# CloudEngineHub/PARC

Hardware: AMD Instinct MI355X
Metric: env-steps/s (higher is better)
Workload: dtype f32; 1 GPU; full step (dynamics + obs/reward/done), 65536 envs total = 65536 per GPU, 5 bundled clips on a square blocky grid, reset of finished envs included; envs_per_gpu=65536, total_envs=65536, dynamics=True, parallelism=env-shard x1, launch=stream launches, library_abi=6

## Files before the change

parc_amd/csrc/parc_env.hip:

```cpp
#include <hip/hip_runtime.h>

#include <cmath>
#include <cstddef>
#include <cstdio>
#include <cstring>
#include <new>
#include <string>
#include <vector>

#include "../../include/parc_env.h"
#include "parc_math.hpp"
#include "parc_dynamics.hpp"
#include "parc_dynamics_coop.hpp"
#include "parc_dynamics_wave.hpp"

using namespace parc;

#define REC_F4 32
#define REC_Q_POS 15
#define REC_Q_CONTACT 16
#define REC_Q_VEL 20

struct HierTables {
    float lt[16][3];
    float lr[16][4];
    int fk_paths[PARC_MAX_FK_PATHS][PARC_MAX_FK_DEPTH];
    int key_ids[8];
    int key_slot[16];
    int parent[16];
    int jtype[16];
    int dof_idx[16];
    float axis[16][4];
};
#define HIER_STAGED_WORDS ((int)(offsetof(HierTables, parent) / 4))

#define TILE_MAX_CELLS 320

struct DevTables {
    HierTables h;
    float tstep[8];
    float joint_err_w[16];
    float dof_err_w[PARC_MAX_DOFS];
    float contact_w[16];
    float pose_term_dist[16];
};

struct MotionMeta {
    int start, nframes;
    float length;
    int loop;
    float dx, dy, dz;
    float fps;
};

struct StepParams {
    int N, B, J, D, K, S, R, M, T;
    int lds_wave_floats;
    int global_obs, off_char;
    int lr_identity;
    int obs_tar, obs_contact;
    int obs_dim, off_dofvel, off_key, off_tar, tar_w, off_tarc, off_cc, off_hf;
    float dt_f, episode_length, min_obs_h, max_obs_h;
    float pose_w, vel_w, root_pos_w, root_vel_w, key_pos_w;
    float root_pos_term_sq, root_rot_term;
    int early_term, pose_term, track_root, track_root_h, tracking, body_pos_from_fk, never_done;
    unsigned fall_mask;
    float term_h;
    const float *hf; int X, Y; float min_x, min_y, dx, dy; int tile_r;
    float rdx, rdy;
    unsigned tile_mul;
    float tstep[8];
    const float4 *records; const MotionMeta *meta; const float *motion_offsets; const float *env_offsets;
    const float *ray_points; const DevTables *tables;
    unsigned char *ema_code;
    unsigned *stamp_out;
    float4 *prep;
    ParcEnvBuffers buf;
};

struct Blend { int i0, i1; float b; };

__device__ __forceinline__ Blend frame_blend(const MotionMeta &m, float t) {
    float phase = t / m.length;
    if (m.loop == PARC_LOOP_WRAP) phase = phase - floorf(phase);
    phase = fminf(fmaxf(phase, 0.f), 1.f);
    float pf = phase * (float)(m.nframes - 1);
    int f0 = (int)pf;
    f0 = max(0, min(f0, m.nframes - 1));
    int f1 = min(f0 + 1, m.nframes - 1);
    Blend r;
    r.b = pf - (float)f0;
    r.i0 = f0 + m.start;
    r.i1 = f1 + m.start;
    return r;
}

__device__ __forceinline__ Q4 joint_dof_to_rot(int type, const float *axis4, const float *dof) {
    if (type == PARC_JOINT_HINGE) return axis_angle_to_quat(mk3(axis4[0], axis4[1], axis4[2]), dof[0]);
    if (type == PARC_JOINT_SPHERICAL) return exp_map_to_quat(mk3(dof[0], dof[1], dof[2]));
    return mk4(0.f, 0.f, 0.f, 1.f);
}

__device__ __forceinline__ void joint_rot_to_dof(int type, const float *axis4, Q4 q, float *out) {
// ... 41 lines not shown

__global__ __launch_bounds__(64) void k_env_prep(const StepParams P, const int64_t *__restrict__ env_ids,
                                                 const int *__restrict__ env_ids32, const int *__restrict__ count_dev, int count) {
    if (count_dev) count = *count_dev;
    const int it = blockIdx.x * 4 + (threadIdx.x >> 4), j = threadIdx.x & 15;
    if (it >= count || j >= P.B) return;
    const int e = env_ids ? (int)env_ids[it] : (env_ids32 ? env_ids32[it] : it);
    const DevTables *__restrict__ T = P.tables;
    float4 *out = P.prep + (size_t)e * 16;
    if (j == 0) {
        const float4 rr = *(const float4 *)(P.buf.char_root_rot + 4 * (size_t)e);
        const float heading = calc_heading(rr);
        const Q4 hinv = heading_quat_inv(heading);
        out[0] = make_float4(cosf(heading), sinf(heading), hinv.z, hinv.w);
    } else {
        const float *dof = P.buf.char_dof_pos + (size_t)e * P.D;
        const int ty = T->h.jtype[j], di = T->h.dof_idx[j];
        Q4 q = mk4(0.f, 0.f, 0.f, 1.f);
        if (ty == PARC_JOINT_HINGE) q = axis_angle_to_quat(mk3(T->h.axis[j][0], T->h.axis[j][1], T->h.axis[j][2]), dof[di]);
        else if (ty == PARC_JOINT_SPHERICAL) q = exp_map_to_quat(mk3(dof[di], dof[di + 1], dof[di + 2]));
        out[j] = q;
    }
}

#ifdef PARC_STAMPS
#define STAMP(i) do { if (lane == 0) s_stamp[i] = __builtin_readcyclecounter(); } while (0)
#else
#define STAMP(i) do { } while (0)
#endif
#define MODE_STEP 0
#define MODE_OBS 1
#define ENVS_PER_BLOCK 4
#define WAVE_SYNC() asm volatile("" ::: "memory")
#define RAY_UNROLL 8

__device__ __forceinline__ float wave_sum(float v) {
#pragma unroll
    for (int off = 32; off >= 1; off >>= 1) v = v + __shfl_xor(v, off, 64);
    return v;
}

template <int CTRL>
__device__ __forceinline__ float dpp_f32(float v) {
    return __int_as_float(__builtin_amdgcn_update_dpp(0, __float_as_int(v), CTRL, 0xf, 0xf, false));
}
__device__ __forceinline__ float row_sum16(float v) {
    v = v + dpp_f32<0x128>(v);
    v = v + dpp_f32<0x124>(v);
    v = v + dpp_f32<0x122>(v);
    v = v + dpp_f32<0x121>(v);
    return v;
}
__device__ __forceinline__ float lane_value(float v, int l) { return __int_as_float(__builtin_amdgcn_readlane(__float_as_int(v), l)); }

template <int MODE, bool MIRROR, bool LOCALROOT = false, bool OBSVAR = false>
__global__ __launch_bounds__(256, 5) void k_env_post(const StepParams P, const int64_t *__restrict__ env_ids,
                                                 const int *__restrict__ env_ids32, const int *__restrict__ count_dev, int count,
                                                 unsigned long long *bump_calls) {
    extern __shared__ __align__(16) float s_obs_all[];
    __shared__ int s_tab_raw[HIER_STAGED_WORDS];
    const HierTables &s_tab = *reinterpret_cast<const HierTables *>(s_tab_raw);
    __shared__ float4 s_q_all[ENVS_PER_BLOCK][8][16];
    __shared__ float4 s_lq_all[ENVS_PER_BLOCK][2][16];
    __shared__ float4 s_fk_all[ENVS_PER_BLOCK][80];
    __shared__ float s_cdofv_all[ENVS_PER_BLOCK][PARC_MAX_DOFS];
    __shared__ float4 s_refvel_all[ENVS_PER_BLOCK][12];
    __shared__ float s_refct_all[ENVS_PER_BLOCK][16];
    __shared__ float s_cfn_all[ENVS_PER_BLOCK][16];
    __shared__ float s_sc_all[ENVS_PER_BLOCK][16];
#ifdef PARC_STAMPS
    __shared__ unsigned long long s_stamp_all[ENVS_PER_BLOCK][16];
#endif
    const int wv = __builtin_amdgcn_readfirstlane((int)(threadIdx.x >> 6));
    const int lane = threadIdx.x & 63;
    const bool GLOBALOBS = OBSVAR && P.global_obs != 0;
    const int oc = OBSVAR ? P.off_char : 0;
    const bool TAROBS = !OBSVAR || P.obs_tar != 0;
    const bool CONTACTOBS = !OBSVAR || P.obs_contact != 0;
    float *s_obs = s_obs_all + (size_t)wv * P.lds_wave_floats;
    float4 (*s_q)[16] = s_q_all[wv];
    float4 (*s_lq)[16] = s_lq_all[wv];
    float4 *s_fk = s_fk_all[wv];
    float4 *s_cbp = s_lq[0];
    float *s_cdofv = s_cdofv_all[wv];
    float4 *s_refvel = s_refvel_all[wv];
    float *s_refct = s_refct_all[wv], *s_cfn = s_cfn_all[wv];
#ifdef PARC_STAMPS
    unsigned long long *s_stamp = s_stamp_all[wv];
#endif
    float *s_tile = (float *)s_fk;
    float4 (*s_br)[16] = reinterpret_cast<float4 (*)[16]>(s_obs + ((P.off_tarc + 3) & ~3));

    if (MODE == MODE_OBS && bump_calls && blockIdx.x == 0 && threadIdx.x == 0) *bump_calls += 1ull;
    if (count_dev) count = *count_dev;
    const int it = blockIdx.x * ENVS_PER_BLOCK + wv;
    if (it >= count) return;
    int e = env_ids ? (int)env_ids[it] : (env_ids32 ? env_ids32[it] : it);
    e = __builtin_amdgcn_readfirstlane(e);
    STAMP(0);

    const int B = P.B, D = P.D, S = P.S, K = P.K, J = P.J;
    const DevTables *__restrict__ T = P.tables;

    float *orow = P.buf.obs + (size_t)e * P.obs_dim;

    constexpr int HW = HIER_STAGED_WORDS;
    constexpr int HN = (HW + 63) / 64;
    int tabreg[HN];
#pragma unroll
    for (int i = 0; i < HN; ++i) { const int w = lane + 64 * i; tabreg[i] = w < HW ? ((const int *)&T->h)[w] : 0; }
    float dofv = 0.f;
    if (lane < D) dofv = P.buf.char_dof_vel[(size_t)e * D + lane];
    float aux0 = 0.f, aux1 = 0.f, aux2 = 0.f;
    {
        const float *src = nullptr;
        if (lane >= 32 && lane < 32 + B) src = P.buf.contact_forces + 3 * ((size_t)e * B + (lane - 32));
        else if (lane == 30) src = P.buf.char_root_vel + 3 * (size_t)e;
        else if (lane == 31) src = P.buf.char_root_ang_vel + 3 * (size_t)e;
        if (src) { aux0 = src[0]; aux1 = src[1]; aux2 = src[2]; }
    }
    const int qi = lane & 15;
    float4 prepq = make_float4(0.f, 0.f, 0.f, 1.f);
    if (lane < 16) prepq = P.prep[(size_t)e * 16 + lane];
    float2 rayp[RAY_UNROLL];
#pragma unroll
    for (int i = 0; i < RAY_UNROLL; ++i) {
        const int r = lane + 64 * i;
        rayp[i] = r < P.R ? ((const float2 *)P.ray_points)[r] : make_float2(0.f, 0.f);
    }

    const int mid = P.buf.motion_ids[e];
    const int tid = P.buf.terrain_ids[e];
    const float toff = P.buf.time_offsets[e];
    int ts = P.buf.timestep[e];
    if (MODE == MODE_STEP) ts += 1;
    const float time = P.dt_f * (float)ts;
    const float mt = time + toff;
    const MotionMeta meta = P.meta[mid];
    const float eox = P.env_offsets[3 * e + 0], eoy = P.env_offsets[3 * e + 1], eoz = P.env_offsets[3 * e + 2];
    const float *mo = P.motion_offsets + 2 * ((size_t)mid * P.T + tid);
    const float offx = mo[0] - eox, offy = mo[1] - eoy;
    const float *crp = P.buf.char_root_pos + 3 * (size_t)e;
    const float *crr = P.buf.char_root_rot + 4 * (size_t)e;
    const V3 root_pos = mk3(crp[0], crp[1], crp[2]);
    const Q4 root_rot = mk4(crr[0], crr[1], crr[2], crr[3]);
    const float gx = root_pos.x + eox, gy = root_pos.y + eoy, gz = root_pos.z + eoz;

    Blend myb;
    {
        const int sid = lane & 7;
        float t = mt;
#pragma unroll
        for (int q = 0; q < PARC_MAX_TAR_STEPS; ++q) t = (sid - 1 == q) ? mt + P.tstep[q] : t;
        myb = frame_blend(meta, t);
    }
    const int last_frame = meta.start + meta.nframes - 1;
    float4 fA[2], fB[2];
    Blend bl[2];
#pragma unroll
    for (int p = 0; p < 2; ++p) {
        const int r = p * 4 + (lane >> 4);
        const int src = max(r - 1, 0);
        bl[p].b = __shfl(myb.b, src, 64);
        bl[p].i0 = __shfl(myb.i0, src, 64);
        bl[p].i1 = min(bl[p].i0 + 1, last_frame);
        fA[p] = make_float4(0.f, 0.f, 0.f, 1.f); fB[p] = fA[p];
        if (r >= 1 && r < 2 + S) {
            fA[p] = P.records[(size_t)bl[p].i0 * REC_F4 + qi];
            fB[p] = P.records[(size_t)bl[p].i1 * REC_F4 + qi];
        }
    }
    float4 cA = make_float4(0.f, 0.f, 0.f, 0.f), cB = cA;
    float cblend = 0.f;
    const int nvel = 2 + (D + 3) / 4;
    {
        const int src = lane < 4 * (1 + S) ? lane >> 2 : 0;
        const float b2b = __shfl(myb.b, src, 64);
        const int b2i0 = __shfl(myb.i0, src, 64), b2i1 = min(b2i0 + 1, last_frame);
        if (lane < 4 * (1 + S)) {
            const int c = lane & 3;
            cblend = b2b;
            cA = P.records[(size_t)b2i0 * REC_F4 + REC_Q_CONTACT + c];
            cB = P.records[(size_t)b2i1 * REC_F4 + REC_Q_CONTACT + c];
        } else if (lane >= 32 && lane < 32 + nvel) {
            cA = P.records[(size_t)b2i0 * REC_F4 + REC_Q_VEL + (lane - 32)];
        }
    }
    const int tr = P.tile_r, TW = 2 * tr + 1, ncell = tr >= 0 ? TW * TW : 0;
    const int ox = min(max(cell_index(gx, P.min_x, P.dx) - tr, -(1 << 22)), 1 << 22), oy = min(max(cell_index(gy, P.min_y, P.dy) - tr, -(1 << 22)), 1 << 22);
    float tilev[5];
#pragma unroll
    for (int i = 0; i < 5; ++i) {
        const int idx = lane + 64 * i;
        tilev[i] = 0.f;
        if (idx < ncell) {
            const int a = (int)(((unsigned)idx * P.tile_mul) >> 16), bq = idx - a * TW;
            const int cx = min(max(ox + a, 0), P.X - 1), cy = min(max(oy + bq, 0), P.Y - 1);
            tilev[i] = P.hf[(size_t)cx * P.Y + cy];
        }
    }

    const float ch = __shfl(prepq.x, 0, 64), sh = __shfl(prepq.y, 0, 64);
    const Q4 hinv = mk4(0.f, 0.f, __shfl(prepq.z, 0, 64), __shfl(prepq.w, 0, 64));
#pragma unroll
    for (int i = 0; i < HN; ++i) { const int w = lane + 64 * i; if (w < HW) s_tab_raw[w] = tabreg[i]; }
    if (lane < D) {
        s_cdofv[lane] = dofv;
        s_obs[P.off_dofvel + lane] = dofv;
    }
    if (OBSVAR && oc && lane == 29) s_obs[0] = root_pos.z;
    if (lane == 30 || lane == 31) {
        const V3 r = GLOBALOBS ? mk3(aux0, aux1, aux2) : quat_rotate(hinv, mk3(aux0, aux1, aux2));
        const int o = oc + (lane == 30 ? 6 : 9);
        s_obs[o + 0] = r.x; s_obs[o + 1] = r.y; s_obs[o + 2] = r.z;
    }
    if (lane >= 32 && lane < 32 + B) {
        const float n = norm3(mk3(aux0, aux1, aux2));
        if (CONTACTOBS) orow[P.off_cc + (lane - 32)] = n > 1e-5f ? 1.f : 0.f;
        s_cfn[lane - 32] = fminf(n, 1.0f);
    }
#pragma unroll
    for (int i = 0; i < 5; ++i) { const int idx = lane + 64 * i; if (idx < ncell) s_tile[idx] = tilev[i]; }
    WAVE_SYNC();
    STAMP(1);

    {
        float *hrow = orow + P.off_hf;
        float *hmirror = MIRROR && P.buf.ray_hfs ? P.buf.ray_hfs + (size_t)e * P.R : nullptr;
        for (int base = 0; base < P.R; base += 64 * RAY_UNROLL) {
            if (base > 0) {
#pragma unroll
                for (int i = 0; i < RAY_UNROLL; ++i) { const int r = base + lane + 64 * i; rayp[i] = r < P.R ? ((const float2 *)P.ray_points)[r] : make_float2(0.f, 0.f); }
            }
            const float tlox = (float)ox, thix = (float)(ox + TW - 1), tloy = (float)oy, thiy = (float)(oy + TW - 1);
            if (tr >= 0) {
                int tix[RAY_UNROLL];
#pragma unroll
                for (int i = 0; i < RAY_UNROLL; ++i) {
                    tix[i] = 0;
                    if (base + 64 * i < P.R) {
                        const float px = (rayp[i].x * ch - rayp[i].y * sh) + gx;
                        const float py = (rayp[i].x * sh + rayp[i].y * ch) + gy;
                        const int a = (int)fminf(fmaxf(cell_float_rcp(px, P.min_x, P.dx, P.rdx), tlox), thix) - ox;
                        const int bq = (int)fminf(fmaxf(cell_float_rcp(py, P.min_y, P.dy, P.rdy), tloy), thiy) - oy;
                        tix[i] = a * TW + bq;
                    }
                    asm volatile("" : "+v"(tix[i]));
                }
                float hv[RAY_UNROLL];
#pragma unroll
                for (int i = 0; i < RAY_UNROLL; ++i) hv[i] = s_tile[tix[i]];
#pragma unroll
                for (int i = 0; i < RAY_UNROLL; ++i) {
                    const int r = base + lane + 64 * i;
                    if (r < P.R) {
                        float h = hv[i] - gz;
                        h = fminf(fmaxf(h, P.min_obs_h), P.max_obs_h);
                        hrow[r] = h;
                        if (hmirror) hmirror[r] = h;
                    }
                }
            } else {
#pragma unroll
                for (int i = 0; i < RAY_UNROLL; ++i) {
                    const int r = base + lane + 64 * i;
                    if (r < P.R) {
                        const float px = (rayp[i].x * ch - rayp[i].y * sh) + gx;
                        const float py = (rayp[i].x * sh + rayp[i].y * ch) + gy;
                        const int ix = cell_index_rcp(px, P.min_x, P.dx, P.rdx), iy = cell_index_rcp(py, P.min_y, P.dy, P.rdy);
                        const int cx = min(max(ix, 0), P.X - 1), cy = min(max(iy, 0), P.Y - 1);
                        float h = P.hf[(size_t)cx * P.Y + cy] - gz;
                        h = fminf(fmaxf(h, P.min_obs_h), P.max_obs_h);
                        hrow[r] = h;
                        if (hmirror) hmirror[r] = h;
                    }
                }
            }
        }
    }
    STAMP(2);

#pragma unroll
    for (int p = 0; p < 2; ++p) {
        const int r = p * 4 + (lane >> 4);
        const int i = qi;
        if (r < 2 + S) {
            float4 res = make_float4(0.f, 0.f, 0.f, 1.f);
            if (r == 0) {
                if (i == 0) res = root_rot;
                else if (i == 15) res = make_float4(root_pos.x, root_pos.y, root_pos.z, 0.f);
                else if (i < B) res = prepq;
            } else {
                const float4 A = fA[p], Bv = fB[p];
                const float bb = bl[p].b;
                if (i == 15) {
                    const float a = 1.0f - bb;
                    res.x = a * A.x + bb * Bv.x;
                    res.y = a * A.y + bb * Bv.y;
                    res.z = a * A.z + bb * Bv.z;
                    res.w = 0.f;
                    if (meta.loop == PARC_LOOP_WRAP) {
                        float t = mt;
#pragma unroll
                        for (int q = 0; q < PARC_MAX_TAR_STEPS; ++q) t = (r - 2 == q) ? mt + P.tstep[q] : t;
                        const float ph = floorf(t / meta.length);
                        res.x = res.x + ph * meta.dx; res.y = res.y + ph * meta.dy; res.z = res.z + ph * meta.dz;
                    }
                    res.x = res.x + offx;
                    res.y = res.y + offy;
                } else if (i < B) {
                    res = slerp_rr(A, Bv, bb);
                }
// ... 327 lines not shown
                te[3] = pe / (float)B;
                te[4] = dve / (float)D;
                te[5] = (fabsf(tv.x - rvx) + fabsf(tv.y - rvy) + fabsf(tv.z - rvz)) / 3.f;
                te[6] = (fabsf(tav.x - rax) + fabsf(tav.y - ray_) + fabsf(tav.z - raz)) / 3.f;
            }
        }
    }
    if (P.body_pos_from_fk && P.buf.char_body_pos && lane < B) {
        float *o = P.buf.char_body_pos + 3 * ((size_t)e * B + lane);
        const float4 v = s_fk[lane];
        o[0] = v.x; o[1] = v.y; o[2] = v.z;
    }
    WAVE_SYNC();
    STAMP(6);

    {
        const int nst = P.off_tarc;
        if ((P.obs_dim & 3) == 0) {
            const float4 *src = (const float4 *)s_obs;
            float4 *dst = (float4 *)orow;
            const int n4 = nst >> 2;
            for (int i = lane; i < n4; i += 64) dst[i] = src[i];
            for (int i = 4 * n4 + lane; i < nst; i += 64) orow[i] = s_obs[i];
        } else {
            for (int i = lane; i < nst; i += 64) orow[i] = s_obs[i];
        }
    }
    STAMP(7);
#ifdef PARC_STAMPS
    WAVE_SYNC();
    if (lane < 7 && P.stamp_out) P.stamp_out[(size_t)e * 8 + lane] = (unsigned)(s_stamp[lane + 1] - s_stamp[lane]);
    if (lane == 7 && P.stamp_out) P.stamp_out[(size_t)e * 8 + 7] = 0;
#endif
}

__device__ __forceinline__ int nonzero_bytes(unsigned v) {
    return ((v & 0xffu) != 0) + ((v & 0xff00u) != 0) + ((v & 0xff0000u) != 0) + ((v & 0xff000000u) != 0);
}

__device__ __forceinline__ void done_scatter_block(const unsigned char *__restrict__ ema_code, const int *__restrict__ motion_ids, int N, int *done_list,
                                                   int *done_key, int *reset_count, int never_done, int b, int nblocks) {
    __shared__ int s_base, s_wave[16];
    const int tid = threadIdx.x, lane = tid & 63, wv = tid >> 6;
    if (tid == 0) s_base = 0;
    __syncthreads();
    {
        const uint4 *src = (const uint4 *)ema_code;
        int c = 0;
        for (int i = tid; i < 64 * b; i += 1024) {
            const uint4 v = src[i];
            c += nonzero_bytes(v.x) + nonzero_bytes(v.y) + nonzero_bytes(v.z) + nonzero_bytes(v.w);
        }
        for (int off = 32; off >= 1; off >>= 1) c += __shfl_xor(c, off, 64);
        if (lane == 0 && c) atomicAdd(&s_base, c);
    }
    const int e = b * 1024 + tid;
    const unsigned char code = e < N ? ema_code[e] : 0;
    const unsigned long long mask = __ballot(code != 0);
    const int prefix = __popcll(mask & ((1ull << lane) - 1ull));
    if (lane == 0) s_wave[wv] = __popcll(mask);
    __syncthreads();
    int woff = 0, total = 0;
    for (int i = 0; i < 16; ++i) { const int c = s_wave[i]; if (i < wv) woff += c; total += c; }
    if (code) {
        const int pos = s_base + woff + prefix;
        done_list[pos] = e;
// ... 933 lines not shown
    HIPCHK(hipMalloc((void **)&d_rp, sizeof(float) * 3 * F));
    HIPCHK(hipMalloc((void **)&d_rr, sizeof(float) * 4 * F));
    HIPCHK(hipMalloc((void **)&d_jr, sizeof(float) * 4 * J * F));
    HIPCHK(hipMalloc((void **)&d_fm, sizeof(int) * F));
    HIPCHK(hipMemcpy(e->d_meta, e->h_meta.data(), sizeof(MotionMeta) * M, hipMemcpyHostToDevice));
    HIPCHK(hipMemcpy(e->d_weights, e->h_weights.data(), sizeof(float) * M, hipMemcpyHostToDevice));
    std::vector<float> ones(M, 1.0f);
    HIPCHK(hipMemcpy(e->d_fail, ones.data(), sizeof(float) * M, hipMemcpyHostToDevice));
    HIPCHK(hipMemcpy(d_rp, c->root_pos_host, sizeof(float) * 3 * F, hipMemcpyHostToDevice));
    HIPCHK(hipMemcpy(d_rr, c->root_rot_host, sizeof(float) * 4 * F, hipMemcpyHostToDevice));
    HIPCHK(hipMemcpy(d_jr, c->joint_rot_host, sizeof(float) * 4 * J * F, hipMemcpyHostToDevice));
    HIPCHK(hipMemcpy(d_fm, frame_motion.data(), sizeof(int) * F, hipMemcpyHostToDevice));
    if (c->contacts_host) {
        HIPCHK(hipMalloc((void **)&d_ct, sizeof(float) * B * F));
        HIPCHK(hipMemcpy(d_ct, c->contacts_host, sizeof(float) * B * F, hipMemcpyHostToDevice));
    }
    PrepParams pp;
    pp.F = (int)F; pp.B = B; pp.J = J; pp.D = e->D; pp.root_pos = d_rp; pp.root_rot = d_rr; pp.joint_rot = d_jr; pp.contacts = d_ct;
    pp.frame_motion = d_fm; pp.meta = e->d_meta; pp.tables = e->d_tab; pp.records = e->d_records;
    hipLaunchKernelGGL(k_motion_prep, dim3((unsigned)((F + 127) / 128)), dim3(128), 0, 0, pp);
    HIPCHK(hipGetLastError());
    HIPCHK(hipDeviceSynchronize());
    (void)hipFree(d_rp); (void)hipFree(d_rr); (void)hipFree(d_jr); (void)hipFree(d_fm);
    if (d_ct) (void)hipFree(d_ct);
    e->M = M; e->F = F; e->have_motions = true;
    e->sp.M = M; e->sp.records = e->d_records; e->sp.meta = e->d_meta;
    return sync_params(e);
}

extern "C" int parc_env_load_terrain(ParcEnv *e, const float *hf, int32_t X, int32_t Y, float min_x, float min_y, float dx, float dy,
                                     const float *motion_offsets, int32_t M, int32_t T) {
    if (!e || !hf || !motion_offsets || X < 1 || Y < 1 || T < 1 || !(dx > 0.f) || !(dy > 0.f)) return fail(PARC_ERR_INVALID, "bad terrain");
    if (!e->have_motions || M != e->M) return fail(PARC_ERR_STATE, "load_motions first; motion_offsets must have one row per motion");
    HIPCHK(hipSetDevice(e->cfg.device));
    if (e->d_hf) (void)hipFree(e->d_hf);
    if (e->d_motion_off) (void)hipFree(e->d_motion_off);
    e->d_hf = nullptr; e->d_motion_off = nullptr;
    HIPCHK(hipMalloc((void **)&e->d_hf, sizeof(float) * (size_t)X * Y));
    HIPCHK(hipMalloc((void **)&e->d_motion_off, sizeof(float) * 2 * (size_t)M * T));
    HIPCHK(hipMemcpy(e->d_hf, hf, sizeof(float) * (size_t)X * Y, hipMemcpyHostToDevice));
    HIPCHK(hipMemcpy(e->d_motion_off, motion_offsets, sizeof(float) * 2 * (size_t)M * T, hipMemcpyHostToDevice));
    StepParams &sp = e->sp;
    sp.hf = e->d_hf; sp.X = X; sp.Y = Y; sp.min_x = min_x; sp.min_y = min_y; sp.dx = dx; sp.dy = dy; sp.T = T;
    sp.rdx = (float)(1.0L / (long double)dx); sp.rdy = (float)(1.0L / (long double)dy);
    sp.motion_offsets = e->d_motion_off;
    e->T = T;
    e->hf_max = hf[0];
    for (size_t q = 1; q < (size_t)X * Y; ++q) e->hf_max = fmaxf(e->hf_max, hf[q]);
    e->hf_min = hf[0];
    for (size_t q = 1; q < (size_t)X * Y; ++q) e->hf_min = fminf(e->hf_min, hf[q]);
    std::vector<float> ray(2 * (size_t)e->R);
    HIPCHK(hipMemcpy(ray.data(), e->d_ray, sizeof(float) * 2 * e->R, hipMemcpyDeviceToHost));
    float rmax = 0.f;
    for (int r = 0; r < e->R; ++r) rmax = fmaxf(rmax, sqrtf(ray[2 * r] * ray[2 * r] + ray[2 * r + 1] * ray[2 * r + 1]));
    int tr = (int)ceilf(rmax / fminf(dx, dy) + 0.01f);
    if ((2 * tr + 1) * (2 * tr + 1) > TILE_MAX_CELLS) tr = -1;
    sp.tile_r = tr;
    if (tr >= 0) {
        const unsigned TW = 2 * tr + 1;
        const unsigned mul = (65536u + TW - 1) / TW;
        for (unsigned idx = 0; idx < TW * TW; ++idx)
            if (((idx * mul) >> 16) != idx / TW) return fail(PARC_ERR_INVALID, "internal: tile index multiplier");
        sp.tile_mul = mul;
    }
    const int stage_pad = (sp.off_tarc + 3) & ~3;
    e->lds_bytes = sizeof(float) * (size_t)stage_pad + (e->cfg.report_tracking_error ? 2 * 16 * sizeof(float4) : 0);
    e->sp.lds_wave_floats = (int)(e->lds_bytes / sizeof(float));
    e->have_terrain = true;
    e->graph_dirty = true;
    return sync_params(e);
}

extern "C" int parc_env_bind_buffers(ParcEnv *e, const ParcEnvBuffers *b) {
    if (!e || !b) return fail(PARC_ERR_INVALID, "null argument");
    const void *req[] = {b->char_root_pos, b->char_root_rot, b->char_root_vel, b->char_root_ang_vel, b->char_dof_pos, b->char_dof_vel,
                         b->contact_forces, b->motion_ids, b->terrain_ids, b->time_offsets, b->timestep, b->obs, b->reward, b->done};
    for (const void *p : req) if (!p) return fail(PARC_ERR_INVALID, "a required buffer is NULL");
    if (!e->cfg.body_pos_from_fk && !b->char_body_pos) return fail(PARC_ERR_INVALID, "char_body_pos is required when body_pos_from_fk == 0");
    if (((uintptr_t)b->obs & 15) != 0) return fail(PARC_ERR_INVALID, "obs must be 16-byte aligned");
    if ((b->ref_root_rot && ((uintptr_t)b->ref_root_rot & 15)) || (b->ref_joint_rot && ((uintptr_t)b->ref_joint_rot & 15)) ||
        ((uintptr_t)b->char_root_rot & 15))
        return fail(PARC_ERR_INVALID, "quaternion buffers must be 16-byte aligned");
    e->sp.buf = *b;
    e->bound = true;
    e->graph_dirty = true;
    return sync_params(e);
}

static int check_ready(ParcEnv *e) {
    if (!e) return fail(PARC_ERR_INVALID, "null env");
    if (!e->bound || !e->have_motions || !e->have_terrain) return fail(PARC_ERR_STATE, "bind_buffers, load_motions and load_terrain must precede this call");
    return PARC_OK;
}

static int launch_dynamics(ParcEnv *e, const float *action_dev, hipStream_t st) {
    if (!e->cfg.enable_dynamics) return PARC_OK;
    if (!action_dev) return fail(PARC_ERR_INVALID, "action is required when enable_dynamics is set");
// ... 26 lines not shown
        hipLaunchKernelGGL(k_curriculum_small, dim3(e->nchunks + e->M), dim3(1024), 0, st, e->d_ema, e->sp.buf.motion_ids, e->N, e->d_done_list,
                           e->d_done_key, e->d_reset_count, e->sp.never_done, e->nchunks, e->d_fail, e->M, e->cfg.fail_rate_ema_weight, e->d_health);
        HIPCHK(hipGetLastError());
        return PARC_OK;
    }
    hipLaunchKernelGGL(k_done_scatter, dim3(e->nchunks), dim3(1024), 0, st, e->d_ema, e->sp.buf.motion_ids, e->N, e->d_done_list,
                       e->d_done_key, e->d_reset_count, e->sp.never_done, e->d_health);
    if (e->M <= 64 && !e->force_ema_leader) {
        hipLaunchKernelGGL(k_fail_rate_ema, dim3(e->M), dim3(1024), 0, st, e->d_done_key, e->d_reset_count, e->d_fail, e->M,
                           e->cfg.fail_rate_ema_weight);
    } else {
        hipLaunchKernelGGL(k_ema_first, dim3((e->N + 255) / 256), dim3(256), 0, st, e->d_done_key, e->d_reset_count, e->d_motion_done);
        hipLaunchKernelGGL(k_ema_leader, dim3((e->N + 3) / 4), dim3(256), 0, st, e->d_done_key, e->d_reset_count, e->d_motion_done, e->d_fail,
                           e->cfg.fail_rate_ema_weight);
    }
    HIPCHK(hipGetLastError());
    return PARC_OK;
}

static bool obs_variant(const ParcEnvConfig &c) { return c.global_obs || c.global_root_height_obs || !c.use_contact_info || !c.enable_tar_obs; }

static bool wants_mirror(const ParcEnvBuffers &b) {
    return b.ref_root_pos || b.ref_root_rot || b.ref_root_vel || b.ref_root_ang_vel || b.ref_joint_rot || b.ref_dof_pos || b.ref_dof_vel ||
           b.ref_body_pos || b.ref_contacts || b.ray_hfs || b.tracking_error;
}

static int launch_post(ParcEnv *e, int mode, const int64_t *ids, int count, hipStream_t st, const int *ids32 = nullptr,
                       const int *count_dev = nullptr, bool prep_done = false, unsigned long long *bump = nullptr) {
    if (count <= 0) return PARC_OK;
    const int grid = (count + ENVS_PER_BLOCK - 1) / ENVS_PER_BLOCK;
    const size_t lds = e->lds_bytes * ENVS_PER_BLOCK;
    if (mode == MODE_STEP && e->cfg.enable_dynamics && e->use_wave) prep_done = true;
    if (!prep_done) hipLaunchKernelGGL(k_env_prep, dim3((count + 3) / 4), dim3(64), 0, st, e->sp, ids, ids32, count_dev, count);
    const bool mirror = wants_mirror(e->sp.buf);
    if (obs_variant(e->cfg)) {
        if (mode == MODE_STEP && !e->sp.track_root) hipLaunchKernelGGL((k_env_post<MODE_STEP, true, true, true>), dim3(grid), dim3(64 * ENVS_PER_BLOCK), lds, st, e->sp, ids, ids32, count_dev, count, bump);
        else if (mode == MODE_STEP) hipLaunchKernelGGL((k_env_post<MODE_STEP, true, false, true>), dim3(grid), dim3(64 * ENVS_PER_BLOCK), lds, st, e->sp, ids, ids32, count_dev, count, bump);
        else hipLaunchKernelGGL((k_env_post<MODE_OBS, true, false, true>), dim3(grid), dim3(64 * ENVS_PER_BLOCK), lds, st, e->sp, ids, ids32, count_dev, count, bump);
    } else if (mode == MODE_STEP && !e->sp.track_root) {
        if (mirror) hipLaunchKernelGGL((k_env_post<MODE_STEP, true, true>), dim3(grid), dim3(64 * ENVS_PER_BLOCK), lds, st, e->sp, ids, ids32, count_dev, count, bump);
        else hipLaunchKernelGGL((k_env_post<MODE_STEP, false, true>), dim3(grid), dim3(64 * ENVS_PER_BLOCK), lds, st, e->sp, ids, ids32, count_dev, count, bump);
    } else if (mode == MODE_STEP) {
        if (mirror) hipLaunchKernelGGL((k_env_post<MODE_STEP, true>), dim3(grid), dim3(64 * ENVS_PER_BLOCK), lds, st, e->sp, ids, ids32, count_dev, count, bump);
        else hipLaunchKernelGGL((k_env_post<MODE_STEP, false>), dim3(grid), dim3(64 * ENVS_PER_BLOCK), lds, st, e->sp, ids, ids32, count_dev, count, bump);
    } else {
        if (mirror) hipLaunchKernelGGL((k_env_post<MODE_OBS, true>), dim3(grid), dim3(64 * ENVS_PER_BLOCK), lds, st, e->sp, ids, ids32, count_dev, count, bump);
        else hipLaunchKernelGGL((k_env_post<MODE_OBS, false>), dim3(grid), dim3(64 * ENVS_PER_BLOCK), lds, st, e->sp, ids, ids32, count_dev, count, bump);
    }

    HIPCHK(hipGetLastError());
    return PARC_OK;
}

extern "C" int parc_env_step(ParcEnv *e, const float *action_dev, void *stream) {
    int rc = check_ready(e);
    if (rc) return rc;
    hipStream_t st = (hipStream_t)stream;
    hipEvent_t *tv = nullptr;
    if (e->timing) {
        if (e->tev_used + 4 > e->tev.size()) {
            const size_t old = e->tev.size();
            e->tev.resize(old + 1024, nullptr);
            for (size_t i = old; i < e->tev.size(); ++i) HIPCHK(hipEventCreate(&e->tev[i]));
        }
        tv = &e->tev[e->tev_used];
        e->tev_used += 4;
// ... 496 lines not shown
    std::vector<float> rec((size_t)e->F * 128);
    HIPCHK(hipMemcpy(rec.data(), e->d_records, rec.size() * sizeof(float), hipMemcpyDeviceToHost));
    for (int64_t f = 0; f < e->F; ++f) {
        const float *v = rec.data() + (size_t)f * 128 + 4 * REC_Q_VEL;
        if (root_vel) for (int c = 0; c < 3; ++c) root_vel[3 * f + c] = v[c];
        if (root_ang_vel) for (int c = 0; c < 3; ++c) root_ang_vel[3 * f + c] = v[4 + c];
        if (dof_vel) for (int d = 0; d < e->D; ++d) dof_vel[(size_t)f * e->D + d] = v[8 + d];
    }
    return PARC_OK;
}

extern "C" const unsigned int *parc_env_health_words(ParcEnv *e) { return (e && e->d_health) ? e->h_health : nullptr; }

extern "C" const char *parc_env_describe(ParcEnv *e) {
    if (!e) return "";
    char b[1024];
    std::string d;
    const bool ctrl_ff = e->cfg.enable_dynamics && e->cfg.dynamics.control_mode != PARC_CTRL_PD;
    const char *dk = !e->cfg.enable_dynamics ? "none" : (e->use_wave ? (ctrl_ff ? "k_dynamics_wave_ff" : "k_dynamics_wave") : (e->use_coop ? "k_dynamics_coop" : "k_dynamics"));
    snprintf(b, sizeof(b), "dynamics_kernel=%s;", dk); d += b;
    if (e->cfg.enable_dynamics) {
        const parcdyn::DynModel &m = e->h_dyn;
        static const char *const ctrl_names[] = {"pd", "vel", "torque", "pd_exp", "pd_1d"};
        snprintf(b, sizeof(b), "control_mode=%s;", ctrl_names[m.ctrl]); d += b;
        snprintf(b, sizeof(b), "envs_per_block=%d;substeps=%d;substep_dt=%.9g;collision_points=%d;collision_segments=%d;kn=%g;dn=%g;dtang=%g;mu=%g;pen_cap=%g;"
                 "manifold_period=%d;spec_m0=%g;spec_tv=%g;spec_max=%g;root_residual=%d;", e->use_wave ? wave_envs_per_block(e->N, e->num_cus) : (e->use_coop ? CO_ENVS : 64),
                 m.nsub, (double)m.dt, m.ncol, m.nseg, (double)m.kn, (double)m.dn, (double)m.dtang, (double)m.mu, (double)m.pen_cap, m.man_period, (double)m.spec_m0,
                 (double)m.spec_tv, (double)m.spec_max, e->d_root_shadow ? 1 : 0);
        d += b;
        if (e->wave_rejected) d += "note=the model does not fit k_dynamics_wave (tree shape or > 32 candidates on a body): general fallback kernel;";
        if (e->use_wave) { snprintf(b, sizeof(b), "manifold_lds_slots=%d+%d+%d+%d;manifold_overflow_slots=%d;", e->h_wave.man_cap[0], e->h_wave.man_cap[1], e->h_wave.man_cap[2], e->h_wave.man_cap[3], WV_MAN_OVF); d += b; }
    }
    const bool small = e->M <= 64 && !e->force_ema_leader && e->N <= CURRICULUM_ONE_LAUNCH_MAX && (e->N & 7) == 0 && !e->force_two_launch_curriculum;
    snprintf(b, sizeof(b), "curriculum=%s;post_kernel=%s;dev_options=%s", small ? "k_curriculum_small" : ((e->M <= 64 && !e->force_ema_leader) ? "k_done_scatter+k_fail_rate_ema" : "k_done_scatter+k_ema_first+k_ema_leader"),
             e->bound ? parc_env_post_kernel(e) : "unbound", e->dev_options_s.empty() ? "none" : e->dev_options_s.c_str());
    d += b;
    e->describe_s = d;
    return e->describe_s.c_str();
}

extern "C" int parc_env_dynamics_timeouts(ParcEnv *e) {
    if (!e) return fail(PARC_ERR_INVALID, "null env");
    unsigned int v = 0;
    HIPCHK(hipSetDevice(e->cfg.device));
    HIPCHK(hipDeviceSynchronize());
    HIPCHK(hipMemcpyFromSymbol(&v, HIP_SYMBOL(parcdyn::g_wave_timeouts), sizeof(v)));
    return (int)(v > 0x7fffffffu ? 0x7fffffffu : v);
}

extern "C" int parc_env_dynamics_manifold_drops(ParcEnv *e) {
    if (!e) return fail(PARC_ERR_INVALID, "null env");
    unsigned int v = 0;
    HIPCHK(hipSetDevice(e->cfg.device));
    HIPCHK(hipDeviceSynchronize());
    HIPCHK(hipMemcpyFromSymbol(&v, HIP_SYMBOL(parcdyn::g_wave_man_drops), sizeof(v)));
    return (int)(v > 0x7fffffffu ? 0x7fffffffu : v);
}

extern "C" float parc_env_last_dynamics_ms(ParcEnv *e) { return e ? e->last_dyn_ms : 0.f; }

extern "C" const char *parc_env_dynamics_kernel(ParcEnv *e) {
    if (!e || !e->cfg.enable_dynamics) return "";
    return e->use_wave ? "k_dynamics_wave" : (e->use_coop ? "k_dynamics_coop" : "k_dynamics");
}

extern "C" const char *parc_env_post_kernel(ParcEnv *e) {
    if (!e || !e->bound) return "";
// ... 221 lines not shown
```

Measured before the change: 98.56 million env-steps/s.

## Split heightfield ray sampling into a separate persistent k_ray_obs kernel

Removes the per-env LDS terrain tile and ray sampling from k_env_post and moves it into a new grid-strided kernel. In the new kernel each wave keeps a chunk of ray points in registers and loops over many envs, prefetching the next env's root data, reading the heightfield directly from global memory and writing with an aligned offset. This is meant to cut register/LDS pressure and per-env ray-point reloads in the main post kernel, and to improve store coalescing. In exchange it adds an extra kernel launch, gives up the LDS tile reuse for terrain reads, and caps terrain size for 32-bit byte addressing.

```diff
diff --git a/parc_amd/csrc/parc_env.hip b/parc_amd/csrc/parc_env.hip
--- a/parc_amd/csrc/parc_env.hip
+++ b/parc_amd/csrc/parc_env.hip
@@ -3,6 +3,7 @@
 #include <cmath>
 #include <cstddef>
 #include <cstdio>
+#include <algorithm>
 #include <cstring>
 #include <new>
 #include <string>
@@ -33,8 +34,6 @@
     float axis[16][4];
 };
 #define HIER_STAGED_WORDS ((int)(offsetof(HierTables, parent) / 4))
-
-#define TILE_MAX_CELLS 320
 
 struct DevTables {
     HierTables h;
@@ -66,9 +65,8 @@
     int early_term, pose_term, track_root, track_root_h, tracking, body_pos_from_fk, never_done;
     unsigned fall_mask;
     float term_h;
-    const float *hf; int X, Y; float min_x, min_y, dx, dy; int tile_r;
+    const float *hf; int X, Y; float min_x, min_y, dx, dy;
     float rdx, rdy;
-    unsigned tile_mul;
     float tstep[8];
     const float4 *records; const MotionMeta *meta; const float *motion_offsets; const float *env_offsets;
     const float *ray_points; const DevTables *tables;
@@ -176,7 +174,7 @@
 #define MODE_OBS 1
 #define ENVS_PER_BLOCK 4
 #define WAVE_SYNC() asm volatile("" ::: "memory")
-#define RAY_UNROLL 8
+#define RAY_CHUNK 7
 
 __device__ __forceinline__ float wave_sum(float v) {
 #pragma unroll
@@ -232,7 +230,6 @@
 #ifdef PARC_STAMPS
     unsigned long long *s_stamp = s_stamp_all[wv];
 #endif
-    float *s_tile = (float *)s_fk;
     float4 (*s_br)[16] = reinterpret_cast<float4 (*)[16]>(s_obs + ((P.off_tarc + 3) & ~3));
 
     if (MODE == MODE_OBS && bump_calls && blockIdx.x == 0 && threadIdx.x == 0) *bump_calls += 1ull;
@@ -266,13 +263,6 @@
     const int qi = lane & 15;
     float4 prepq = make_float4(0.f, 0.f, 0.f, 1.f);
     if (lane < 16) prepq = P.prep[(size_t)e * 16 + lane];
-    float2 rayp[RAY_UNROLL];
-#pragma unroll
-    for (int i = 0; i < RAY_UNROLL; ++i) {
-        const int r = lane + 64 * i;
-        rayp[i] = r < P.R ? ((const float2 *)P.ray_points)[r] : make_float2(0.f, 0.f);
-    }
-
     const int mid = P.buf.motion_ids[e];
     const int tid = P.buf.terrain_ids[e];
     const float toff = P.buf.time_offsets[e];
@@ -281,14 +271,13 @@
     const float time = P.dt_f * (float)ts;
     const float mt = time + toff;
     const MotionMeta meta = P.meta[mid];
-    const float eox = P.env_offsets[3 * e + 0], eoy = P.env_offsets[3 * e + 1], eoz = P.env_offsets[3 * e + 2];
+    const float eox = P.env_offsets[3 * e + 0], eoy = P.env_offsets[3 * e + 1];
     const float *mo = P.motion_offsets + 2 * ((size_t)mid * P.T + tid);
     const float offx = mo[0] - eox, offy = mo[1] - eoy;
     const float *crp = P.buf.char_root_pos + 3 * (size_t)e;
     const float *crr = P.buf.char_root_rot + 4 * (size_t)e;
     const V3 root_pos = mk3(crp[0], crp[1], crp[2]);
     const Q4 root_rot = mk4(crr[0], crr[1], crr[2], crr[3]);
-    const float gx = root_pos.x + eox, gy = root_pos.y + eoy, gz = root_pos.z + eoz;
 
     Blend myb;
     {
@@ -330,21 +319,6 @@
             cA = P.records[(size_t)b2i0 * REC_F4 + REC_Q_VEL + (lane - 32)];
         }
     }
-    const int tr = P.tile_r, TW = 2 * tr + 1, ncell = tr >= 0 ? TW * TW : 0;
-    const int ox = min(max(cell_index(gx, P.min_x, P.dx) - tr, -(1 << 22)), 1 << 22), oy = min(max(cell_index(gy, P.min_y, P.dy) - tr, -(1 << 22)), 1 << 22);
-    float tilev[5];
-#pragma unroll
-    for (int i = 0; i < 5; ++i) {
-        const int idx = lane + 64 * i;
-        tilev[i] = 0.f;
-        if (idx < ncell) {
-            const int a = (int)(((unsigned)idx * P.tile_mul) >> 16), bq = idx - a * TW;
-            const int cx = min(max(ox + a, 0), P.X - 1), cy = min(max(oy + bq, 0), P.Y - 1);
-            tilev[i] = P.hf[(size_t)cx * P.Y + cy];
-        }
-    }
-
-    const float ch = __shfl(prepq.x, 0, 64), sh = __shfl(prepq.y, 0, 64);
     const Q4 hinv = mk4(0.f, 0.f, __shfl(prepq.z, 0, 64), __shfl(prepq.w, 0, 64));
 #pragma unroll
     for (int i = 0; i < HN; ++i) { const int w = lane + 64 * i; if (w < HW) s_tab_raw[w] = tabreg[i]; }
@@ -363,65 +337,9 @@
         if (CONTACTOBS) orow[P.off_cc + (lane - 32)] = n > 1e-5f ? 1.f : 0.f;
         s_cfn[lane - 32] = fminf(n, 1.0f);
     }
-#pragma unroll
-    for (int i = 0; i < 5; ++i) { const int idx = lane + 64 * i; if (idx < ncell) s_tile[idx] = tilev[i]; }
     WAVE_SYNC();
     STAMP(1);
 
-    {
-        float *hrow = orow + P.off_hf;
-        float *hmirror = MIRROR && P.buf.ray_hfs ? P.buf.ray_hfs + (size_t)e * P.R : nullptr;
-        for (int base = 0; base < P.R; base += 64 * RAY_UNROLL) {
-            if (base > 0) {
-#pragma unroll
-                for (int i = 0; i < RAY_UNROLL; ++i) { const int r = base + lane + 64 * i; rayp[i] = r < P.R ? ((const float2 *)P.ray_points)[r] : make_float2(0.f, 0.f); }
-            }
-            const float tlox = (float)ox, thix = (float)(ox + TW - 1), tloy = (float)oy, thiy = (float)(oy + TW - 1);
-            if (tr >= 0) {
-                int tix[RAY_UNROLL];
-#pragma unroll
-                for (int i = 0; i < RAY_UNROLL; ++i) {
-                    tix[i] = 0;
-                    if (base + 64 * i < P.R) {
-                        const float px = (rayp[i].x * ch - rayp[i].y * sh) + gx;
-                        const float py = (rayp[i].x * sh + rayp[i].y * ch) + gy;
-                        const int a = (int)fminf(fmaxf(cell_float_rcp(px, P.min_x, P.dx, P.rdx), tlox), thix) - ox;
-                        const int bq = (int)fminf(fmaxf(cell_float_rcp(py, P.min_y, P.dy, P.rdy), tloy), thiy) - oy;
-                        tix[i] = a * TW + bq;
-                    }
-                    asm volatile("" : "+v"(tix[i]));
-                }
-                float hv[RAY_UNROLL];
-#pragma unroll
-                for (int i = 0; i < RAY_UNROLL; ++i) hv[i] = s_tile[tix[i]];
-#pragma unroll
-                for (int i = 0; i < RAY_UNROLL; ++i) {
-                    const int r = base + lane + 64 * i;
-                    if (r < P.R) {
-                        float h = hv[i] - gz;
-                        h = fminf(fmaxf(h, P.min_obs_h), P.max_obs_h);
-                        hrow[r] = h;
-                        if (hmirror) hmirror[r] = h;
-                    }
-                }
-            } else {
-#pragma unroll
-                for (int i = 0; i < RAY_UNROLL; ++i) {
-                    const int r = base + lane + 64 * i;
-                    if (r < P.R) {
-                        const float px = (rayp[i].x * ch - rayp[i].y * sh) + gx;
-                        const float py = (rayp[i].x * sh + rayp[i].y * ch) + gy;
-                        const int ix = cell_index_rcp(px, P.min_x, P.dx, P.rdx), iy = cell_index_rcp(py, P.min_y, P.dy, P.rdy);
-                        const int cx = min(max(ix, 0), P.X - 1), cy = min(max(iy, 0), P.Y - 1);
-                        float h = P.hf[(size_t)cx * P.Y + cy] - gz;
-                        h = fminf(fmaxf(h, P.min_obs_h), P.max_obs_h);
-                        hrow[r] = h;
-                        if (hmirror) hmirror[r] = h;
-                    }
-                }
-            }
-        }
-    }
     STAMP(2);
 
 #pragma unroll
@@ -815,6 +733,79 @@
     if (lane < 7 && P.stamp_out) P.stamp_out[(size_t)e * 8 + lane] = (unsigned)(s_stamp[lane + 1] - s_stamp[lane]);
     if (lane == 7 && P.stamp_out) P.stamp_out[(size_t)e * 8 + 7] = 0;
 #endif
+}
+
+struct RayEnv { int e; float ox, oy, oz, px, py, pz, ch, sh; };
+__device__ __forceinline__ RayEnv ray_env_load(const StepParams &P, const int64_t *__restrict__ env_ids, const int *__restrict__ env_ids32, int it) {
+    RayEnv h;
+    h.e = __builtin_amdgcn_readfirstlane(env_ids ? (int)env_ids[it] : (env_ids32 ? env_ids32[it] : it));
+    const float *eo = P.env_offsets + 3 * (size_t)h.e, *crp = P.buf.char_root_pos + 3 * (size_t)h.e;
+    h.ox = eo[0]; h.oy = eo[1]; h.oz = eo[2];
+    h.px = crp[0]; h.py = crp[1]; h.pz = crp[2];
+    const float2 hd = *(const float2 *)(P.prep + (size_t)h.e * 16);
+    h.ch = hd.x; h.sh = hd.y;
+    return h;
+}
+
+__global__ __launch_bounds__(256) void k_ray_obs(const StepParams P, const int64_t *__restrict__ env_ids, const int *__restrict__ env_ids32,
+                                                 const int *__restrict__ count_dev, int count) {
+    if (count_dev) count = *count_dev;
+    const int lane = threadIdx.x & 63;
+    const int wv = __builtin_amdgcn_readfirstlane((int)(threadIdx.x >> 6));
+    const int nw = (int)gridDim.x * 4, first = (int)blockIdx.x * 4 + wv;
+    if (first >= count) return;
+    const int shift = (32 - (P.off_hf & 31)) & 31;
+    const float2 *__restrict__ pts = (const float2 *)P.ray_points;
+    for (int base = -shift; base < P.R; base += 64 * RAY_CHUNK) {
+        float2 rp[RAY_CHUNK];
+#pragma unroll
+        for (int i = 0; i < RAY_CHUNK; ++i) {
+            const int r = base + 64 * i + lane;
+            rp[i] = (r >= 0 && r < P.R) ? pts[r] : make_float2(0.f, 0.f);
+        }
+        int it = first;
+        RayEnv cur = ray_env_load(P, env_ids, env_ids32, it);
+        for (;;) {
+            const int nit = it + nw;
+            const bool more = nit < count;
+            RayEnv nxt = cur;
+            if (more) nxt = ray_env_load(P, env_ids, env_ids32, nit);
+            const float gx = cur.px + cur.ox, gy = cur.py + cur.oy, gz = cur.pz + cur.oz;
+            const float ch = cur.ch, sh = cur.sh;
+            char *hrow = (char *)(P.buf.obs + (size_t)cur.e * P.obs_dim + P.off_hf);
+            char *hmirror = P.buf.ray_hfs ? (char *)(P.buf.ray_hfs + (size_t)cur.e * P.R) : nullptr;
+            unsigned off[RAY_CHUNK];
+#pragma unroll
+            for (int i = 0; i < RAY_CHUNK; ++i) { off[i] = 4u * (unsigned)(base + 64 * i + lane); asm volatile("" : "+v"(off[i])); }
+            float hv[RAY_CHUNK];
+#pragma unroll
+            for (int i = 0; i < RAY_CHUNK; ++i) {
+                hv[i] = 0.f;
+                if (base + 64 * i < P.R) {
+                    const float px = (rp[i].x * ch - rp[i].y * sh) + gx;
+                    const float py = (rp[i].x * sh + rp[i].y * ch) + gy;
+                    const int ix = cell_index_rcp(px, P.min_x, P.dx, P.rdx), iy = cell_index_rcp(py, P.min_y, P.dy, P.rdy);
+                    const int cx = min(max(ix, 0), P.X - 1), cy = min(max(iy, 0), P.Y - 1);
+                    hv[i] = *(const float *)((const char *)P.hf + 4u * (__umul24((unsigned)cx, (unsigned)P.Y) + (unsigned)cy));
+                }
+            }
+#pragma unroll
+            for (int i = 0; i < RAY_CHUNK; ++i) {
+                const int r = base + 64 * i + lane;
+                hv[i] = fminf(fmaxf(hv[i] - gz, P.min_obs_h), P.max_obs_h);
+                if (r >= 0 && r < P.R) *(float *)(hrow + off[i]) = hv[i];
+            }
+            if (hmirror) {
+#pragma unroll
+                for (int i = 0; i < RAY_CHUNK; ++i) {
+                    const int r = base + 64 * i + lane;
+                    if (r >= 0 && r < P.R) *(float *)(hmirror + off[i]) = hv[i];
+                }
+            }
+            if (!more) break;
+            cur = nxt; it = nit;
+        }
+    }
 }
 
 __device__ __forceinline__ int nonzero_bytes(unsigned v) {
@@ -1814,6 +1805,8 @@
                                      const float *motion_offsets, int32_t M, int32_t T) {
     if (!e || !hf || !motion_offsets || X < 1 || Y < 1 || T < 1 || !(dx > 0.f) || !(dy > 0.f)) return fail(PARC_ERR_INVALID, "bad terrain");
     if (!e->have_motions || M != e->M) return fail(PARC_ERR_STATE, "load_motions first; motion_offsets must have one row per motion");
+    if (X >= (1 << 24) || Y >= (1 << 24) || (long long)X * Y > (1ll << 30))
+        return fail(PARC_ERR_INVALID, "terrain: at most 2^24 - 1 cells per axis and 2^30 cells (k_ray_obs addresses a cell with a 32-bit byte offset)");
     HIPCHK(hipSetDevice(e->cfg.device));
     if (e->d_hf) (void)hipFree(e->d_hf);
     if (e->d_motion_off) (void)hipFree(e->d_motion_off);
@@ -1831,20 +1824,6 @@
     for (size_t q = 1; q < (size_t)X * Y; ++q) e->hf_max = fmaxf(e->hf_max, hf[q]);
     e->hf_min = hf[0];
     for (size_t q = 1; q < (size_t)X * Y; ++q) e->hf_min = fminf(e->hf_min, hf[q]);
-    std::vector<float> ray(2 * (size_t)e->R);
-    HIPCHK(hipMemcpy(ray.data(), e->d_ray, sizeof(float) * 2 * e->R, hipMemcpyDeviceToHost));
-    float rmax = 0.f;
-    for (int r = 0; r < e->R; ++r) rmax = fmaxf(rmax, sqrtf(ray[2 * r] * ray[2 * r] + ray[2 * r + 1] * ray[2 * r + 1]));
-    int tr = (int)ceilf(rmax / fminf(dx, dy) + 0.01f);
-    if ((2 * tr + 1) * (2 * tr + 1) > TILE_MAX_CELLS) tr = -1;
-    sp.tile_r = tr;
-    if (tr >= 0) {
-        const unsigned TW = 2 * tr + 1;
-        const unsigned mul = (65536u + TW - 1) / TW;
-        for (unsigned idx = 0; idx < TW * TW; ++idx)
-            if (((idx * mul) >> 16) != idx / TW) return fail(PARC_ERR_INVALID, "internal: tile index multiplier");
-        sp.tile_mul = mul;
-    }
     const int stage_pad = (sp.off_tarc + 3) & ~3;
     e->lds_bytes = sizeof(float) * (size_t)stage_pad + (e->cfg.report_tracking_error ? 2 * 16 * sizeof(float4) : 0);
     e->sp.lds_wave_floats = (int)(e->lds_bytes / sizeof(float));
@@ -1937,6 +1916,7 @@
     const size_t lds = e->lds_bytes * ENVS_PER_BLOCK;
     if (mode == MODE_STEP && e->cfg.enable_dynamics && e->use_wave) prep_done = true;
     if (!prep_done) hipLaunchKernelGGL(k_env_prep, dim3((count + 3) / 4), dim3(64), 0, st, e->sp, ids, ids32, count_dev, count);
+    hipLaunchKernelGGL(k_ray_obs, dim3(std::min(grid, 8 * std::max(e->num_cus, 1))), dim3(256), 0, st, e->sp, ids, ids32, count_dev, count);
     const bool mirror = wants_mirror(e->sp.buf);
     if (obs_variant(e->cfg)) {
         if (mode == MODE_STEP && !e->sp.track_root) hipLaunchKernelGGL((k_env_post<MODE_STEP, true, true, true>), dim3(grid), dim3(64 * ENVS_PER_BLOCK), lds, st, e->sp, ids, ids32, count_dev, count, bump);
@@ -2499,7 +2479,7 @@
         if (e->use_wave) { snprintf(b, sizeof(b), "manifold_lds_slots=%d+%d+%d+%d;manifold_overflow_slots=%d;", e->h_wave.man_cap[0], e->h_wave.man_cap[1], e->h_wave.man_cap[2], e->h_wave.man_cap[3], WV_MAN_OVF); d += b; }
     }
     const bool small = e->M <= 64 && !e->force_ema_leader && e->N <= CURRICULUM_ONE_LAUNCH_MAX && (e->N & 7) == 0 && !e->force_two_launch_curriculum;
-    snprintf(b, sizeof(b), "curriculum=%s;post_kernel=%s;dev_options=%s", small ? "k_curriculum_small" : ((e->M <= 64 && !e->force_ema_leader) ? "k_done_scatter+k_fail_rate_ema" : "k_done_scatter+k_ema_first+k_ema_leader"),
+    snprintf(b, sizeof(b), "curriculum=%s;post_kernel=%s;ray_kernel=k_ray_obs;dev_options=%s", small ? "k_curriculum_small" : ((e->M <= 64 && !e->force_ema_leader) ? "k_done_scatter+k_fail_rate_ema" : "k_done_scatter+k_ema_first+k_ema_leader"),
              e->bound ? parc_env_post_kernel(e) : "unbound", e->dev_options_s.empty() ? "none" : e->dev_options_s.c_str());
     d += b;
     e->describe_s = d;
```

Result: slower. 96.54 million env-steps/s (-2.1%).
